# smartroboticslab/okvis2

Measured on AMD Instinct MI355X. Metric: front-end stereo-frames/s (detect+describe+match), 752x480 stereo, higher is better.
Workload: dtype u8/int32 (detect, describe, Hamming) + f64 (match gate); 1 GPU; EuRoC-shaped 752x480 stereo, euroc.yaml front-end params (radius 38, thr 150, <=700 kpts, match thr 60); lanes_per_gpu=1, score_kernels_serialised_across_lanes=False, stereo_frames_per_launch=3072, distinct_frames=256, content=corners, feed=device, cameras_per_multiframe=2, parallelism=frames sharded over 1 GPU(s), no collective

## Files before the change

okvis2_amd/csrc/describe_setup_dev.h:

```cpp
#pragma once
#include "okvfe_internal.h"

namespace okvfe {

__device__ __forceinline__ bool camera_aware_matrix(const float* __restrict__ rays,
                                                    const float* __restrict__ jac, int w, float fu,
                                                    const float dir[3], float kx, float ky,
                                                    float M[4]) {
  const int u = (int)(kx + 0.5f), v = (int)(ky + 0.5f);
  const float* r = rays + ((size_t)v * w + u) * 3;
  const float* J = jac + ((size_t)v * w + u) * 6;
  const float r0 = r[0], r1 = r[1], r2 = r[2];
  if (r0 == 0.0f && r1 == 0.0f && r2 == 0.0f) return false;
  float ey0 = 0.f, ey1 = 0.f, ey2 = 0.f, n2 = 0.0f;
#pragma unroll
  for (int c = 0; c < 3; ++c) {
    const float g0 = c == 0 ? dir[0] : (c == 1 ? 0.0f : 1.0f);
    const float g1 = c == 0 ? dir[1] : (c == 1 ? 1.0f : 0.0f);
    const float g2 = c == 0 ? dir[2] : 0.0f;
    if (c > 0 && n2 >= 1.0e-12f) break;
    float gr = g0 * r0;
    float t = g1 * r1;
    gr = gr + t;
    t = g2 * r2;
    gr = gr + t;
    t = gr * r0; ey0 = g0 - t;
    t = gr * r1; ey1 = g1 - t;
    t = gr * r2; ey2 = g2 - t;
    n2 = ey0 * ey0;
    t = ey1 * ey1;
    n2 = n2 + t;
    t = ey2 * ey2;
    n2 = n2 + t;
  }
  if (!(n2 >= 1.0e-12f)) return false;
  const float n = sqrtf(n2);
  ey0 = ey0 / n;
  ey1 = ey1 / n;
  ey2 = ey2 / n;
  float t1, t2;
  t1 = ey1 * r2; t2 = ey2 * r1; const float ex0 = t1 - t2;
  t1 = ey2 * r0; t2 = ey0 * r2; const float ex1 = t1 - t2;
  t1 = ey0 * r1; t2 = ey1 * r0; const float ex2 = t1 - t2;
  float s;
  s = J[0] * ex0; t1 = J[1] * ex1; s = s + t1; t1 = J[2] * ex2; s = s + t1; M[0] = s / fu;
  s = J[0] * ey0; t1 = J[1] * ey1; s = s + t1; t1 = J[2] * ey2; s = s + t1; M[1] = s / fu;
  s = J[3] * ex0; t1 = J[4] * ex1; s = s + t1; t1 = J[5] * ex2; s = s + t1; M[2] = s / fu;
  s = J[3] * ey0; t1 = J[4] * ey1; s = s + t1; t1 = J[5] * ey2; s = s + t1; M[3] = s / fu;
  return true;
}

template <int MAXB2>
__device__ __forceinline__ bool extra_sample_value(const uint8_t* __restrict__ im, int w, int h, float xf, float yf,
                                                   float sigma_half, int scaling, int scaling2, int* value) {
  const float x_1 = xf - sigma_half, x1 = xf + sigma_half;
  const float y_1 = yf - sigma_half, y1 = yf + sigma_half;
  if (!(x_1 >= 0.0f && y_1 >= 0.0f && x1 < (float)(w - 1) && y1 < (float)(h - 1))) return false;
  const int x_left = (int)(x_1 + 0.5f), y_top = (int)(y_1 + 0.5f);
  const int x_right = (int)(x1 + 0.5f), y_bottom = (int)(y1 + 0.5f);
  float r_x_1 = (float)x_left - x_1;  r_x_1 = r_x_1 + 0.5f;
  float r_y_1 = (float)y_top - y_1;   r_y_1 = r_y_1 + 0.5f;
  float r_x1 = x1 - (float)x_right;   r_x1 = r_x1 + 0.5f;
  float r_y1 = y1 - (float)y_bottom;  r_y1 = r_y1 + 0.5f;
  const float fs = (float)scaling;
  float t;
  t = r_x_1 * r_y_1; const int A = (int)(t * fs);
  t = r_x1 * r_y_1;  const int B = (int)(t * fs);
  t = r_x1 * r_y1;   const int C = (int)(t * fs);
  t = r_x_1 * r_y1;  const int D = (int)(t * fs);
  const int r_x_1_i = (int)(r_x_1 * fs), r_y_1_i = (int)(r_y_1 * fs);
  const int r_x1_i = (int)(r_x1 * fs), r_y1_i = (int)(r_y1 * fs);
  const int bw = x_right - x_left, bh = y_bottom - y_top;
  if (bw > MAXB2 || bh > MAXB2) return false;
  constexpr int NDW = (3 + MAXB2) / 4 + 1;
  const int b = x_left & 3;
  const uint8_t* p0 = im + (size_t)y_top * w + (x_left & ~3);
  auto byte_at = [&](const uint32_t (&r)[NDW], int pos) -> int {
    uint32_t v = r[0];
#pragma unroll
    for (int j = 1; j < NDW; ++j) v = (pos >> 2) == j ? r[j] : v;
    return (int)((v >> (8 * (pos & 3))) & 0xFFu);
  };
  uint32_t msk[NDW];
#pragma unroll
  for (int j = 0; j < NDW; ++j) {
    int lo = b + 1 - 4 * j, hi = b + bw - 4 * j;
    lo = lo < 0 ? 0 : (lo > 4 ? 4 : lo);
    hi = hi < 0 ? 0 : (hi > 4 ? 4 : hi);
    const uint32_t mlo = lo >= 4 ? 0xFFFFFFFFu : ((1u << (8 * lo)) - 1u);
    const uint32_t mhi = hi >= 4 ? 0xFFFFFFFFu : ((1u << (8 * hi)) - 1u);
    msk[j] = mhi & ~mlo;
  }
  int upper = 0, middle = 0, left = 0, right = 0, bottom = 0, pl_t = 0, pr_t = 0, pl_b = 0, pr_b = 0;
  constexpr int kChunk = 5;
#pragma unroll
  for (int c0 = 0; c0 <= MAXB2; c0 += kChunk) {
    uint32_t d[kChunk][NDW];
#pragma unroll
    for (int r = 0; r < kChunk; ++r) {
      const int dy = c0 + r;
      if (dy <= MAXB2) {
        const uint32_t* q = reinterpret_cast<const uint32_t*>(p0 + (size_t)(dy < bh ? dy : bh) * w);
#pragma unroll
        for (int j = 0; j < NDW; ++j) d[r][j] = q[j];
      }
    }
#pragma unroll
    for (int r = 0; r < kChunk; ++r) {
      const int dy = c0 + r;
      if (dy <= MAXB2) {
        const int pl = byte_at(d[r], b), pr = byte_at(d[r], b + bw);
        int in = 0;
#pragma unroll
        for (int j = 0; j < NDW; ++j) in += (int)__builtin_amdgcn_sad_u8(d[r][j] & msk[j], 0u, 0u);
        if (dy == 0) {
          pl_t = pl;
          pr_t = pr;
          upper = in;
        } else if (dy < bh) {
          left += pl;
          right += pr;
          middle += in;
        } else if (dy == bh) {
          pl_b = pl;
          pr_b = pr;
          bottom = in;
        }
      }
    }
  }
  int ret = A * pl_t;
  ret += B * pr_t;
  ret += C * pr_b;
  ret += D * pl_b;
  ret += upper * r_y_1_i + middle * scaling + left * r_x_1_i + right * r_x1_i + bottom * r_y1_i;
  *value = (ret + scaling2 / 2) / scaling2;
  return true;
}

__device__ __forceinline__ bool extra_sample_one(const Pattern* __restrict__ pat, const uint8_t* __restrict__ im, int w,
                                                 int h, int extra_box, int e, const float M[4], float kx, float ky,
                                                 uint8_t* __restrict__ slot_bytes) {
  const float px = pat->px[e], py = pat->py[e], sg = pat->sigma_half[e];
  float a = M[0] * px, b2 = M[1] * py;
  a = a + b2;
  const float xf = kx + a;
  float c = M[2] * px, d2 = M[3] * py;
  c = c + d2;
  const float yf = ky + c;
  int v = 0;
  const bool ok = extra_box <= 4
                      ? extra_sample_value<4>(im, w, h, xf, yf, sg, pat->box_scaling[e], pat->box_scaling2[e], &v)
                      : extra_sample_value<9>(im, w, h, xf, yf, sg, pat->box_scaling[e], pat->box_scaling2[e], &v);
  *reinterpret_cast<int*>(slot_bytes + 24 + 4 * e) = v;
  return ok;
}

__device__ __forceinline__ void describe_setup_one(const DescribeSetup& ds, int w, int h, int img, size_t slot,
                                                   const okvfe_keypoint& kp) {
  const ImageParams ip = ds.prm[img];
  int scale = 0;
  if (ds.scales) {
    for (int i = 1; i < kPatternScales; ++i) scale += kp.size >= ds.scales->size_from[i] ? 1 : 0;
  }
// ... 51 lines not shown
```

okvis2_amd/csrc/k_select.hip:

```cpp
#include <mutex>
#include "describe_setup_dev.h"
#include <type_traits>

#include "select_common_dev.h"

namespace okvfe {
namespace {

constexpr int kLazyTabBytes = 32 * 32 * 4;
constexpr int kLazyThreads = 256;
constexpr int kLazyBinCap = 4;
#ifndef OKVFE_LAZY_BLOCKMAX
#define OKVFE_LAZY_BLOCKMAX 1024
#endif
#ifndef OKVFE_LAZY_WAVES
#define OKVFE_LAZY_WAVES 6
#endif
constexpr int kLazyBlockMax = OKVFE_LAZY_BLOCKMAX;
constexpr int kLazySurvPerWave = kLazyBlockMax / 4;
__host__ __device__ inline size_t lazy_align16(size_t v) { return (v + 15) & ~(size_t)15; }
__host__ __device__ inline size_t lazy_lds_bytes(int bins_x, int bins_y) {
  const size_t nbins = (size_t)(bins_x + 2) * (bins_y + 2);
  return (size_t)kLazyTabBytes + lazy_align16(nbins * 4) + nbins * kLazyBinCap * 8 + (size_t)kLazyBlockMax * 8 +
         4 * 64 * 4;
}

__device__ __forceinline__ void lds_barrier() {
  asm volatile("s_waitcnt lgkmcnt(0)\n\ts_barrier" ::: "memory");
}

#ifdef OKVFE_LAB
__device__ unsigned long long g_lazy_prof[16];
#define OKVFE_LAZY_TICK(var) const unsigned long long var = __builtin_amdgcn_s_memrealtime()
#else
#define OKVFE_LAZY_TICK(var)
#endif
constexpr int kFuseBins = 496;
constexpr int kFuseUnroll = 8;
constexpr int kFuseFirst = 20;
constexpr int kFuseSched = 40;
__device__ __forceinline__ int fuse_bin(int32_t score) {
  if (score <= 0) return kFuseBins - 1;
  const uint32_t s = (uint32_t)score;
  const int e = 31 - __clz(s);
  const int b = e >= 4 ? (e << 4) | (int)((s >> (e - 4)) & 15u) : (int)s;
  return (kFuseBins - 1) - b;
}
template <bool SORTS>
__global__ __launch_bounds__(kLazyThreads) __attribute__((amdgpu_waves_per_eu(OKVFE_LAZY_WAVES, 8))) void select_lazy_kernel(
    const int32_t* __restrict__ scores, ScoreLayout layout, int w, int h, const Candidate* __restrict__ cand, int cand_cap,
    const int32_t* __restrict__ cand_count, uint64_t* sort_ws, int ws_stride,
    float radius, int max_kpts, const float* __restrict__ lut, int bins_x, int bins_y, int cap,
    okvfe_keypoint* __restrict__ kps, int kp_cap, int32_t* __restrict__ kp_count, uint2* __restrict__ spill_ws,
    size_t spill_stride, int bin_cap, int round_cap, DescribeSetup setup, const uint8_t* __restrict__ images) {
  extern __shared__ __attribute__((aligned(16))) unsigned char smem_raw[];
  __shared__ int s_kept;
  __shared__ int s_spill;
  __shared__ int s_surv[2][4];
  __shared__ uint32_t s_sched[kFuseSched + 2];
  __shared__ int s_nsched, s_max, s_cnt;
  __shared__ unsigned long long s_kmin, s_kmax;
  const int bpitch = bins_x + 2;
  const int nbins = bpitch * (bins_y + 2);
  float* tab = reinterpret_cast<float*>(smem_raw);
  unsigned char* q0 = smem_raw + kLazyTabBytes;
  uint32_t* head = reinterpret_cast<uint32_t*>(q0);
  q0 += lazy_align16((size_t)nbins * 4);
  uint4* slot4 = reinterpret_cast<uint4*>(q0);
  q0 += (size_t)nbins * kLazyBinCap * 8;
  uint64_t* surv = reinterpret_cast<uint64_t*>(q0);
  float* part = reinterpret_cast<float*>(q0 + (size_t)kLazyBlockMax * 8);
  const int tid = threadIdx.x;
  const int wave = __builtin_amdgcn_readfirstlane(tid >> 6);
  const int lane = tid & 63;
  const int img = blockIdx.x;
  int n = cand_count[img];
  n = n > cand_cap ? 0 : n;
  uint64_t* keys = sort_ws + (size_t)img * ws_stride;
  okvfe_keypoint* out = kps + (size_t)img * kp_cap;
  uint2* spill = spill_ws + (size_t)img * spill_stride;
  int kept = 0;
  OKVFE_LAZY_TICK(t_start);
#ifdef OKVFE_LAB
  unsigned long long t_pa = t_start, t_pb = t_start, t_p0 = t_start, t_init = t_start, t_blocks = t_start, t_pref = 0, t_mark = 0, t_walk = 0, t_acc = 0, t_ins = 0, t_w0 = 0, t_w1 = 0, t_w2 = 0;
  int n_surv = 0, n_rounds = 0;
#endif
  if (n > 0) {
    for (int i = tid; i < 32 * 32; i += kLazyThreads) {
      const int dx = i & 31, dy = i >> 5;
      tab[i] = (dx <= 15 && dy <= 15) ? lut[(dy + 15) * 31 + (dx + 15)] : 0.0f;
    }
    for (int i = tid; i < nbins; i += kLazyThreads) head[i] = 0u;
    for (int i = tid; i < nbins * 2; i += kLazyThreads)
      slot4[i] = make_uint4((16u << 23) | (16u << 2), 0u, (16u << 23) | (16u << 2), 0u);
    if (tid == 0) {
      s_kept = 0;
      s_spill = 0;
      if constexpr (SORTS) s_max = INT_MIN;
    }
    if constexpr (SORTS) {
      for (int i = tid; i <= kFuseBins; i += kLazyThreads) reinterpret_cast<uint32_t*>(surv)[i] = 0u;
    }
    const Candidate* crec = cand + (size_t)img * cand_cap;
    int32_t scv0[SORTS ? kFuseFirst : 1];
    uint32_t pyx0[SORTS ? kFuseFirst : 1];
    if constexpr (SORTS) {
#pragma unroll
      for (int u = 0; u < kFuseFirst; ++u) {
        const int i = tid + u * kLazyThreads;
        const Candidate c = i < n ? crec[i] : Candidate{0, 0, INT_MIN};
        scv0[u] = c.score;
        pyx0[u] = ((uint32_t)c.y << 16) | (uint32_t)c.x;
      }
    }
    const float scaling = (float)(15.0 / (double)radius);
    float max_score = 1.0f;
    if constexpr (!SORTS) max_score = (float)(0x7FFFFFFF - (int32_t)(keys[0] >> 32));
    auto make_rec = [&](uint64_t k) {
      const int score = 0x7FFFFFFF - (int32_t)(k >> 32);
      const int y = (int)((k >> 16) & 0xFFFF), x = (int)(k & 0xFFFF);
      const float fy = (float)y * scaling;
      const float fx = (float)x * scaling;
      const int cy = (int)(fy + 16.0f);
      const int cx = (int)(fx + 16.0f);
      const float q = (float)score / max_score;
      const float nsc1 = sqrtf(sqrtf(q)) * 255.0f;
      return make_uint4(((uint32_t)cy << 16) | (uint32_t)cx, __float_as_uint(nsc1), (uint32_t)(k & 0xFFFFFFFFu),
                        (uint32_t)score);
    };
    const uint32_t tab_addr = (uint32_t)(uintptr_t)(__attribute__((address_space(3))) float*)tab;
    auto waddr_of = [&](uint32_t A, uint32_t code, uint32_t levbits) {
      const uint32_t a = __builtin_amdgcn_sad_u16(A, code, tab_addr);
      return levbits != 0u ? a : tab_addr;
    };
    auto term = [&](uint32_t waddr, uint32_t levbits) {
      return ceilf(*reinterpret_cast<__attribute__((address_space(3))) const float*>((uintptr_t)waddr) *
                   __uint_as_float(levbits));
    };
    auto bins3 = [&](const int b[3], const uint32_t A[3], int half) {
      uint4 s3[3];
#pragma unroll
      for (int k = 0; k < 3; ++k) s3[k] = slot4[2 * b[k] + half];
      uint32_t wa[6];
#pragma unroll
      for (int k = 0; k < 3; ++k) {
        wa[2 * k] = waddr_of(A[k], half == 0 ? s3[k].x & ~1u : s3[k].x, s3[k].y);
        wa[2 * k + 1] = waddr_of(A[k], s3[k].z, s3[k].w);
      }
      float f = 0.0f;
#pragma unroll
      for (int k = 0; k < 3; ++k) f += term(wa[2 * k], s3[k].y) + term(wa[2 * k + 1], s3[k].w);
      return f;
    };
    auto spill_terms = [&](int cx, int cy) {
      float f = 0.0f;
      const int ns = s_spill;
      for (int i = 0; i < ns; ++i) {
        const uint2 p = spill[i];
        const int dx = cx - (int)(p.x & 0xFFFF), dy = cy - (int)(p.x >> 16);
        const int adx = dx < 0 ? -dx : dx, ady = dy < 0 ? -dy : dy;
        if (adx <= 15 && ady <= 15) f += ceilf(tab[(ady << 5) | adx] * __uint_as_float(p.y));
      }
      return f;
    };
    const int first = (wave + 1) & 3;
    const int nch = first == 0 ? 3 : 2;
    int hoff[3];
    uint32_t aoff[3];
#pragma unroll
    for (int k = 0; k < 3; ++k) {
      const int c = first + 4 * k < 9 ? first + 4 * k : first;
      const int ox = (c % 3) - 1, oy = (c / 3) - 1;
      hoff[k] = oy * bpitch + ox;
      aoff[k] = ((uint32_t)(-16 * oy) << 23) + ((uint32_t)(-16 * ox) << 2);
    }
    const int limit = min(min(max_kpts, kp_cap), cap);
    uint64_t* my_surv = surv + wave * kLazySurvPerWave;
    auto prefilter_key = [&](uint64_t kthis, bool valid) -> bool {
          uint4 rec = make_rec(kthis);
          if (!valid) rec.x = 0u;
          const int cx = (int)(rec.x & 0xFFFF), cy = (int)(rec.x >> 16);
          const float level = __uint_as_float(rec.y);
          const int bin = ((cy >> 4) + 1) * bpitch + ((cx >> 4) + 1);
          const uint32_t lx = (uint32_t)(cx & 15), ly = (uint32_t)(cy & 15);
          const uint32_t A0 = ((ly + 16u) << 23) | ((lx + 16u) << 2);
          float occf = 0.0f;
          {
            bool more = false;
            auto batch = [&](auto first, auto count) {
              constexpr int B0 = decltype(first)::value, NB = decltype(count)::value;
              uint32_t A[NB];
              uint4 sb[NB];
#pragma unroll
              for (int q = 0; q < NB; ++q) {
                const int b = B0 + q;
// ... 196 lines not shown
#pragma unroll
        for (int t = 0; t < 4; ++t) {
          const int i = lo + 64 * t + lane;
          kr[t] = i < hi ? keys[i] : 0ull;
        }
      };
      uint64_t kcur[4] = {0ull, 0ull, 0ull, 0ull}, knxt[4];
      int blen = 64, par = 0;
      for (int a = 0; a < n; a += blen, blen = min(2 * blen, kLazyBlockMax), par ^= 1) {
        const int e = min(a + blen, n);
#ifdef OKVFE_LAB
        t_mark = __builtin_amdgcn_s_memrealtime();
#endif
        int my_cnt = 0;
        if (a == 0) {
          const int q = (e - a + 3) >> 2;
          const int lo = wave * q, hi = min(lo + q, e - a);
          for (int c = lo + lane; c < hi; c += 64) my_surv[c - lo] = keys[c];
          my_cnt = hi > lo ? hi - lo : 0;
        } else {
          const int q = blen >> 2;
          const int lo = a + wave * q, hi = min(lo + q, e);
#pragma unroll
          for (int t = 0; t < 4; ++t) {
            const int c0 = lo + 64 * t;
            if (c0 >= hi) break;
            const uint64_t kthis = kcur[t];
            const bool pass = prefilter_key(kthis, c0 + lane < hi);
            const unsigned long long m = __ballot(pass);
            if (pass) my_surv[my_cnt + __popcll(m & ((1ull << lane) - 1ull))] = kthis;
            my_cnt += __popcll(m);
          }
        }
        load_quarter(a + blen, min(2 * blen, kLazyBlockMax), knxt);
        if (lane == 0) s_surv[par][wave] = my_cnt;
        lds_barrier();
        const int c0n = s_surv[par][0], c1n = c0n + s_surv[par][1], c2n = c1n + s_surv[par][2],
                  total = c2n + s_surv[par][3];
#ifdef OKVFE_LAB
        n_surv += total;
        t_pref += __builtin_amdgcn_s_memrealtime() - t_mark;
#endif
        windows(total, [&](int g) {
          int li = 0, lo = g;
          if (g >= c2n) { li = 3; lo = g - c2n; }
          else if (g >= c1n) { li = 2; lo = g - c1n; }
          else if (g >= c0n) { li = 1; lo = g - c0n; }
          return surv[li * kLazySurvPerWave + lo];
        });
        if (kept >= limit) break;
#pragma unroll
        for (int t = 0; t < 4; ++t) kcur[t] = knxt[t];
      }
    } else {
      uint32_t* hist = reinterpret_cast<uint32_t*>(surv);
      __syncthreads();
#ifdef OKVFE_LAB
      t_p0 = __builtin_amdgcn_s_memrealtime();
#endif
      {
        int mx = INT_MIN;
#pragma unroll
        for (int u = 0; u < kFuseFirst; ++u) {
          if (tid + u * kLazyThreads < n) {
            atomicAdd(&hist[fuse_bin(scv0[u])], 1u);
            mx = max(mx, scv0[u]);
          }
        }
        for (int base = tid + kFuseFirst * kLazyThreads; base < n; base += 8 * kLazyThreads) {
          int32_t scv[8];
#pragma unroll
          for (int u = 0; u < 8; ++u) {
            const int i = base + u * kLazyThreads;
            scv[u] = i < n ? crec[i].score : INT_MIN;
          }
#pragma unroll
          for (int u = 0; u < 8; ++u) {
            if (base + u * kLazyThreads < n) {
              atomicAdd(&hist[fuse_bin(scv[u])], 1u);
              mx = max(mx, scv[u]);
            }
          }
        }
#pragma unroll
        for (int d = 32; d > 0; d >>= 1) mx = max(mx, __shfl_xor(mx, d));
        if (lane == 0) atomicMax(&s_max, mx);
      }
      __syncthreads();
#ifdef OKVFE_LAB
      t_pa = __builtin_amdgcn_s_memrealtime();
#endif
      max_score = (float)s_max;
      if (wave == 0) {
        uint32_t v[8], sum = 0;
#pragma unroll
        for (int k = 0; k < 8; ++k) {
          const int idx = lane * 8 + k;
          v[k] = idx < kFuseBins ? hist[idx] : 0u;
          sum += v[k];
        }
        uint32_t inc = sum;
#pragma unroll
        for (int d = 1; d < 64; d <<= 1) {
          const uint32_t t = __shfl_up(inc, d);
          if (lane >= d) inc += t;
        }
        uint32_t run = inc - sum;
        __builtin_amdgcn_wave_barrier();
#pragma unroll
        for (int k = 0; k < 8; ++k) {
          const int idx = lane * 8 + k;
          if (idx <= kFuseBins) hist[idx] = run;
          run += v[k];
        }
        __builtin_amdgcn_wave_barrier();
        int pos = 0, b = 0, k = 0;
        uint32_t target = min(64u, (uint32_t)round_cap);
        while (pos < n && k < kFuseSched) {
          int x_last = b - 1;
          for (int base = b; base < kFuseBins; base += 64) {
            const int idx = base + lane;
            const uint32_t ve = idx < kFuseBins ? hist[idx + 1] : 0xFFFFFFFFu;
            const bool ok = idx < kFuseBins && ve - (uint32_t)pos <= target;
            const int c = __popcll(__ballot(ok));
            x_last += c;
            if (c < 64) break;
          }
          int e = x_last >= b ? (int)hist[x_last + 1] : pos;
          if (e == pos) {
            for (int base = b; base < kFuseBins; base += 64) {
              const int idx = base + lane;
              const bool gt = idx < kFuseBins && (int)hist[idx + 1] > pos;
              const unsigned long long m = __ballot(gt);
              if (m != 0ull) {
                x_last = base + (int)__ffsll((long long)m) - 1;
                break;
              }
            }
            e = (int)hist[x_last + 1];
          }
          if (lane == 0) s_sched[k] = (uint32_t)e;
          ++k;
          pos = e;
          b = x_last + 1;
          target = min(2u * target, (uint32_t)round_cap);
        }
        if (pos < n) {
          if (lane == 0) s_sched[k] = (uint32_t)n;
          ++k;
        }
        if (lane == 0) s_nsched = k;
      }
      __syncthreads();
#ifdef OKVFE_LAB
      t_pb = __builtin_amdgcn_s_memrealtime();
#endif
#pragma unroll
      for (int u = 0; u < kFuseFirst; ++u) {
        if (tid + u * kLazyThreads < n) {
          const uint32_t p = atomicAdd(&hist[fuse_bin(scv0[u])], 1u);
          keys[p] = ((uint64_t)(uint32_t)(0x7FFFFFFF - scv0[u]) << 32) | pyx0[u];
        }
      }
      for (int base = tid + kFuseFirst * kLazyThreads; base < n; base += kFuseUnroll * kLazyThreads) {
        Candidate cv[kFuseUnroll];
#pragma unroll
        for (int u = 0; u < kFuseUnroll; ++u) {
          const int i = base + u * kLazyThreads;
          cv[u] = i < n ? crec[i] : Candidate{0, 0, 0};
        }
#pragma unroll
        for (int u = 0; u < kFuseUnroll; ++u) {
          if (base + u * kLazyThreads < n) {
            const uint32_t p = atomicAdd(&hist[fuse_bin(cv[u].score)], 1u);
            keys[p] = make_key(cv[u]);
          }
        }
      }
      __syncthreads();
#ifdef OKVFE_LAB
      t_init = __builtin_amdgcn_s_memrealtime();
#endif
      const int nsched = s_nsched;
      uint64_t kcur[4] = {0ull, 0ull, 0ull, 0ull}, knxt[4] = {0ull, 0ull, 0ull, 0ull};
      auto load_chunk = [&](int c0, int m, uint64_t kr[4]) {
        const int q = (m + 3) >> 2;
        const int lo = c0 + wave * q, hi = min(lo + q, c0 + m);
#pragma unroll
        for (int t = 0; t < 4; ++t) {
          const int i = lo + 64 * t + lane;
          kr[t] = i < hi ? keys[i] : 0ull;
        }
      };
      int cpos = 0, j = 0, par = 0;
      bool have_next = false;
      bool refining = false;
      int r_base = 0, r_m = 0, r_rem = 0;
      uint64_t r_lo = 0ull;
      while (true) {
        int cnt = 0;
#ifdef OKVFE_LAB
        t_mark = __builtin_amdgcn_s_memrealtime();
#endif
        if (!refining) {
          if (j >= nsched) break;
          const int e = (int)s_sched[j];
          const int m = e - cpos;
          ++j;
          if (m > round_cap) {
            refining = true;
            r_base = cpos; r_m = m; r_rem = m; r_lo = 0ull;
            cpos = e;
            have_next = false;
            continue;
          }
          if (have_next) {
#pragma unroll
            for (int t = 0; t < 4; ++t) kcur[t] = knxt[t];
          } else {
            load_chunk(cpos, m, kcur);
          }
          cnt = m;
          cpos = e;
          have_next = false;
        } else {
          uint64_t hi = ~0ull;
          if (r_rem > round_cap) {
            if (tid == 0) {
              s_kmin = ~0ull;
              s_kmax = 0ull;
            }
            __syncthreads();
            unsigned long long mn = ~0ull, mxk = 0ull;
            for (int i = tid; i < r_m; i += kLazyThreads) {
              const unsigned long long k = keys[r_base + i];
              if (k >= r_lo) {
                mn = k < mn ? k : mn;
                mxk = k > mxk ? k : mxk;
              }
            }
#pragma unroll
            for (int d = 32; d > 0; d >>= 1) {
              const unsigned long long a1 = __shfl_xor(mn, d), a2 = __shfl_xor(mxk, d);
              mn = a1 < mn ? a1 : mn;
              mxk = a2 > mxk ? a2 : mxk;
            }
            if (lane == 0) {
              atomicMin(&s_kmin, mn);
              atomicMax(&s_kmax, mxk);
            }
            __syncthreads();
            const unsigned long long kmin = s_kmin, range = s_kmax - kmin;
            int sh = range < 256ull ? 0 : (64 - __clzll((long long)range)) - 8;
            uint32_t* sub = reinterpret_cast<uint32_t*>(part);
            while (true) {
              sub[tid] = 0u;
              __syncthreads();
              for (int i = tid; i < r_m; i += kLazyThreads) {
                const unsigned long long k = keys[r_base + i];
                if (k >= r_lo) {
                  const unsigned long long d = (k - kmin) >> sh;
                  if (d < 256ull) atomicAdd(&sub[(int)d], 1u);
                }
              }
              __syncthreads();
              uint32_t v4[4], sum = 0;
#pragma unroll
              for (int k = 0; k < 4; ++k) {
                v4[k] = sub[lane * 4 + k];
                sum += v4[k];
              }
              uint32_t inc = sum;
#pragma unroll
              for (int d = 1; d < 64; d <<= 1) {
                const uint32_t t = __shfl_up(inc, d);
                if (lane >= d) inc += t;
              }
              uint32_t run = inc - sum;
              int nfit = 0;
#pragma unroll
              for (int k = 0; k < 4; ++k) {
                run += v4[k];
                nfit += __popcll(__ballot(run <= (uint32_t)round_cap));
              }
              __syncthreads();
              if (nfit == 0 && sh > 0) {
                sh = sh >= 8 ? sh - 8 : 0;
                continue;
              }
              hi = kmin + ((unsigned long long)(nfit > 0 ? nfit : 1) << sh);
              break;
            }
          }
          if (tid == 0) s_cnt = 0;
          __syncthreads();
          for (int i0 = 0; i0 < r_m; i0 += kLazyThreads) {
            const int i = i0 + tid;
            const unsigned long long k = i < r_m ? keys[r_base + i] : 0ull;
            const bool pred = i < r_m && k >= r_lo && k < hi;
            const unsigned long long m = __ballot(pred);
            if (m != 0ull) {
              int base = 0;
              if (lane == 0) base = atomicAdd(&s_cnt, __popcll(m));
              base = __builtin_amdgcn_readfirstlane(base);
              const int at = base + __popcll(m & ((1ull << lane) - 1ull));
              if (pred && at < kLazyBlockMax) surv[at] = k;
            }
          }
          __syncthreads();
          const int got = s_cnt;
          cnt = got < kLazyBlockMax ? got : kLazyBlockMax;
          {
            const int q = (cnt + 3) >> 2;
            const int lo = wave * q, hi_i = min(lo + q, cnt);
#pragma unroll
            for (int t = 0; t < 4; ++t) {
              const int i = lo + 64 * t + lane;
              kcur[t] = i < hi_i ? surv[i] : 0ull;
            }
          }
          __syncthreads();
          r_rem -= got;
          r_lo = hi;
          if (r_rem <= 0 || got == 0) refining = false;
        }
        int my_cnt = 0;
        {
          const int q = (cnt + 3) >> 2;
          const int lo = wave * q, hi_i = min(lo + q, cnt);
#pragma unroll
          for (int t = 0; t < 4; ++t) {
            const int c0 = lo + 64 * t;
            if (c0 >= hi_i) break;
            const uint64_t kthis = kcur[t];
            const bool valid = c0 + lane < hi_i;
            const bool pass = kept > 0 ? prefilter_key(kthis, valid) : valid;
            const unsigned long long m = __ballot(pass);
            if (pass) my_surv[my_cnt + __popcll(m & ((1ull << lane) - 1ull))] = kthis;
            my_cnt += __popcll(m);
          }
        }
        if (!refining && j < nsched) {
          const int m2 = (int)s_sched[j] - cpos;
          if (m2 <= round_cap) {
            load_chunk(cpos, m2, knxt);
            have_next = true;
          }
        }
        int* racc = reinterpret_cast<int*>(part);
        racc[tid] = 0;
        if (lane == 0) s_surv[par][wave] = my_cnt;
        lds_barrier();
        const int c0n = s_surv[par][0], c1n = c0n + s_surv[par][1], c2n = c1n + s_surv[par][2],
                  total = c2n + s_surv[par][3];
        par ^= 1;
#ifdef OKVFE_LAB
        n_surv += total;
        ++n_rounds;
#endif
        auto list_key = [&](int g) {
          int li = 0, lo = g;
          if (g >= c2n) { li = 3; lo = g - c2n; }
          else if (g >= c1n) { li = 2; lo = g - c1n; }
          else if (g >= c0n) { li = 1; lo = g - c0n; }
          return surv[li * kLazySurvPerWave + lo];
        };
        auto list_len = [&](int w2) { return w2 == 0 ? c0n : (w2 == 1 ? c1n - c0n : (w2 == 2 ? c2n - c1n : total - c2n)); };
        if (total <= kLazyThreads / 2) {
          const int per = total <= 64 ? 1 : 2;
          const int g = total <= 64 ? lane : (tid & 127);
          const int w0 = total <= 64 ? wave : 2 * (wave >> 1);
          const uint64_t mykey = g < total ? list_key(g) : ~0ull;
          int r = 0;
          for (int w2 = w0; w2 < w0 + per; ++w2) {
            const uint64_t* lst = surv + w2 * kLazySurvPerWave;
            const int c = list_len(w2);
#pragma unroll 8
            for (int jj = 0; jj < c; ++jj) r += lst[jj] < mykey ? 1 : 0;
          }
          if (g < total && r != 0) atomicAdd(&racc[g], r);
          lds_barrier();
          if (w0 == 0 && g < total) surv[racc[g]] = mykey;
          lds_barrier();
        } else {
          const int nu = (total + kLazyThreads - 1) / kLazyThreads;
          uint64_t mykey[4];
          int rank[4];
#pragma unroll
          for (int u = 0; u < 4; ++u) {
            const int g = tid + u * kLazyThreads;
            mykey[u] = (u < nu && g < total) ? list_key(g) : ~0ull;
            rank[u] = 0;
          }
#pragma unroll
          for (int w2 = 0; w2 < 4; ++w2) {
            const uint64_t* lst = surv + w2 * kLazySurvPerWave;
            const int c = list_len(w2);
            if (nu <= 1) {
#pragma unroll 8
              for (int jj = 0; jj < c; ++jj) rank[0] += lst[jj] < mykey[0] ? 1 : 0;
            } else {
              for (int jj = 0; jj < c; ++jj) {
                const uint64_t k2 = lst[jj];
#pragma unroll
                for (int u = 0; u < 4; ++u) rank[u] += k2 < mykey[u] ? 1 : 0;
              }
            }
          }
          lds_barrier();
#pragma unroll
          for (int u = 0; u < 4; ++u)
            if (u < nu && tid + u * kLazyThreads < total) surv[rank[u]] = mykey[u];
          lds_barrier();
        }
#ifdef OKVFE_LAB
        t_pref += __builtin_amdgcn_s_memrealtime() - t_mark;
#endif
        windows(total, [&](int g) { return surv[g]; });
        if (kept >= limit) break;
      }
    }
  }
  __syncthreads();
#ifdef OKVFE_LAB
  t_blocks = __builtin_amdgcn_s_memrealtime();
#endif
  for (int i = tid; i < kept; i += kLazyThreads) {
    okvfe_keypoint kp = out[i];
    const int u = (int)kp.x, v = (int)kp.y;
    int32_t patch[9];
    if (images) {
      harris_scores_3x3(images + (size_t)img * w * h, w, h, u, v, patch);
    } else {
      const int32_t* sc = scores + (size_t)img * layout.pitch * h;
#pragma unroll
      for (int dy = -1; dy <= 1; ++dy)
#pragma unroll
        for (int dx = -1; dx <= 1; ++dx)
          patch[(dy + 1) * 3 + (dx + 1)] = sc[score_index(layout, u + dx, v + dy)];
    }
    float ddx, ddy;
    subpixel2d(patch, &ddx, &ddy);
    kp.x = (float)u + ddx;
    kp.y = (float)v + ddy;
    kp.response = (float)kp.class_id;
    kp.class_id = -1;
    out[i] = kp;
    if (setup.pat) describe_setup_one(setup, w, h, img, (size_t)img * kp_cap + i, kp);
  }
  if (tid == 0) kp_count[img] = kept;
#ifdef OKVFE_LAB
  __syncthreads();
  if (tid == 0 && img == 0) {
    const unsigned long long t_end = __builtin_amdgcn_s_memrealtime();
    atomicAdd(&g_lazy_prof[0], 1ull);
    atomicAdd(&g_lazy_prof[1], t_init - t_start);
    atomicAdd(&g_lazy_prof[2], t_blocks - t_init);
    atomicAdd(&g_lazy_prof[3], t_end - t_blocks);
    atomicAdd(&g_lazy_prof[4], t_end - t_start);
    atomicAdd(&g_lazy_prof[5], t_pref);
    atomicAdd(&g_lazy_prof[6], (unsigned long long)n_surv);
    atomicAdd(&g_lazy_prof[7], (unsigned long long)n);
    atomicAdd(&g_lazy_prof[8], t_walk);
    atomicAdd(&g_lazy_prof[9], t_acc);
    atomicAdd(&g_lazy_prof[10], t_ins);
    atomicAdd(&g_lazy_prof[11], (unsigned long long)n_rounds);
    atomicAdd(&g_lazy_prof[12], t_p0 - t_start);
    atomicAdd(&g_lazy_prof[13], t_pa - t_p0);
    atomicAdd(&g_lazy_prof[14], t_pb - t_pa);
    atomicAdd(&g_lazy_prof[15], t_init - t_pb);
  }
#endif
}

}


constexpr int kListChunk = 128;
constexpr int kListLutBytes = 64 * 64 * 4;
__device__ __forceinline__ uint32_t lds_u32(uint32_t addr) {
  return *reinterpret_cast<__attribute__((address_space(3))) const uint32_t*>((uintptr_t)addr);
}
__device__ __forceinline__ float lds_f32(uint32_t addr) {
  return *reinterpret_cast<__attribute__((address_space(3))) const float*>((uintptr_t)addr);
}
__host__ __device__ inline size_t list_lds_bytes(int bins_x, int bins_y, int cap) {
  return (size_t)kListLutBytes + lazy_align16((size_t)(bins_x + 2) * (bins_y + 2) * 4) +
         2 * lazy_align16((size_t)(cap + 1) * 4) + (size_t)kListChunk * 16 + 4 * 64 * 4;
}

__global__ __launch_bounds__(kLazyThreads) __attribute__((amdgpu_waves_per_eu(6, 8))) void select_list_kernel(
    const int32_t* __restrict__ scores, ScoreLayout layout, int w, int h, int cand_cap,
    const int32_t* __restrict__ cand_count, const uint64_t* __restrict__ sort_ws, int ws_stride,
    float radius, int max_kpts, const float* __restrict__ lut, int bins_x, int bins_y, int cap,
    okvfe_keypoint* __restrict__ kps, int kp_cap, int32_t* __restrict__ kp_count, DescribeSetup setup,
    const uint8_t* __restrict__ images) {
  extern __shared__ __attribute__((aligned(16))) unsigned char smem_raw[];
  __shared__ int s_kept;
  const int bpitch = bins_x + 2;
  const int nbins = bpitch * (bins_y + 2);
  const size_t cap4 = lazy_align16((size_t)(cap + 1) * 4);
  float* lut_s = reinterpret_cast<float*>(smem_raw);
  unsigned char* q0 = smem_raw + kListLutBytes;
  uint32_t* head = reinterpret_cast<uint32_t*>(q0);
  q0 += lazy_align16((size_t)nbins * 4);
  uint32_t* link = reinterpret_cast<uint32_t*>(q0);
  float* pnsc = reinterpret_cast<float*>(q0 + cap4);
  uint4* recs = reinterpret_cast<uint4*>(q0 + 2 * cap4);
  float* part = reinterpret_cast<float*>(q0 + 2 * cap4 + (size_t)kListChunk * 16);
  const int tid = threadIdx.x;
  const int wave = __builtin_amdgcn_readfirstlane(tid >> 6);
  const int lane = tid & 63;
  const int img = blockIdx.x;
  int n = cand_count[img];
  n = n > cand_cap ? 0 : n;
  const uint64_t* keys = sort_ws + (size_t)img * ws_stride;
  okvfe_keypoint* out = kps + (size_t)img * kp_cap;
  int kept = 0;
  if (n > 0) {
    for (int i = tid; i < 64 * 64; i += kLazyThreads) {
      const int dx = (i & 63) - 32, dy = (i >> 6) - 32;
      const bool in = dx >= -15 && dx <= 15 && dy >= -15 && dy <= 15;
      lut_s[i] = in ? lut[(dy + 15) * 31 + (dx + 15)] : 0.0f;
    }
    const uint32_t link_addr = (uint32_t)(uintptr_t)(__attribute__((address_space(3))) uint32_t*)link;
    const uint32_t end_addr = link_addr + 4u * (uint32_t)cap;
    const uint32_t nsc_delta = (uint32_t)cap4;
    const uint32_t lut_addr = (uint32_t)(uintptr_t)(__attribute__((address_space(3))) float*)lut_s;
    for (int i = tid; i < nbins; i += kLazyThreads) head[i] = end_addr;
    if (tid == 0) {
      pnsc[cap] = 0.0f;
      link[cap] = (end_addr >> 2) << 16;
// ... 99 lines not shown
            if (!pass) cm = 0ull;
            unsigned long long nb = 0ull;
            while (__any(cm != 0ull)) {
              const int el = cm != 0ull ? (int)__ffsll((long long)cm) - 1 : lane;
              const uint32_t exy = (uint32_t)__builtin_amdgcn_ds_bpermute(el << 2, (int)rec.x);
              if (cm != 0ull) {
                cm &= cm - 1ull;
                const uint32_t ddx = (uint32_t)(cx - (int)(exy & 0xFFFF) + 15);
                const uint32_t ddy = (uint32_t)(cy - (int)(exy >> 16) + 15);
                nb |= (ddx <= 30u && ddy <= 30u) ? (1ull << el) : 0ull;
              }
            }
            while (rem != 0ull) {
              const bool in = ((rem >> lane) & 1ull) != 0ull;
              const bool ready = in && (nb & rem) == 0ull;
              const unsigned long long rdy = __ballot(ready);
              const unsigned long long accn = __ballot(ready && pass);
              accm |= accn;
              rem &= ~rdy;
              unsigned long long m = (in && !ready) ? (nb & accn) : 0ull;
              while (__any(m != 0ull)) {
                const int jl = m != 0ull ? (int)__ffsll((long long)m) - 1 : lane;
                const uint32_t jxy = (uint32_t)__builtin_amdgcn_ds_bpermute(jl << 2, (int)rec.x);
                const float jnsc = __int_as_float(__builtin_amdgcn_ds_bpermute(jl << 2, __float_as_int(nsc)));
                if (m != 0ull) {
                  m &= m - 1ull;
                  const int dx = cx - (int)(jxy & 0xFFFF), dy = cy - (int)(jxy >> 16);
                  occ += (int)ceilf(lut_s[((dy + 32) << 6) | (dx + 32)] * jnsc);
                }
              }
              if (in && !ready) pass = !(level < (float)(occ > 255 ? 255 : occ));
              rem &= __ballot(pass);
            }
            nacc = __popcll(accm);
          } else {
            while (rem != 0 && kept + nacc < limit) {
              const int f = (int)__ffsll((long long)rem) - 1;
              accm |= 1ull << f;
              ++nacc;
              const uint32_t wxy = (uint32_t)__builtin_amdgcn_readlane((int)rec.x, f);
              const float wnsc = __int_as_float(__builtin_amdgcn_readlane(__float_as_int(nsc), f));
              const int dx = cx - (int)(wxy & 0xFFFF), dy = cy - (int)(wxy >> 16);
              const bool near = pass && lane > f && (dx < 0 ? -dx : dx) <= 15 && (dy < 0 ? -dy : dy) <= 15;
              if (__any(near)) {
                if (near) {
                  occ += (int)ceilf(lut_s[((dy + 32) << 6) | (dx + 32)] * wnsc);
                  pass = !(level < (float)(occ > 255 ? 255 : occ));
                }
                rem &= __ballot(pass) & ~(((2ull << f) - 1ull));
              } else {
                rem &= rem - 1;
              }
            }
          }
          if ((accm >> lane) & 1) {
            const int slot = kept + __popcll(accm & ((1ull << lane) - 1ull));
            const uint32_t addr = link_addr + 4u * (uint32_t)slot;
            const uint32_t prev = atomicExch(&head[bin], addr);
            link[slot] = (lcode << 2) | ((prev >> 2) << 16);
            pnsc[slot] = nsc;
            okvfe_keypoint kp;
            kp.x = (float)(int)(rec.z & 0xFFFF);
            kp.y = (float)(int)(rec.z >> 16);
            kp.size = 12.0f;
            kp.angle = -1.0f;
            kp.response = (float)(int32_t)rec.w;
            kp.octave = 0;
            kp.class_id = (int32_t)rec.w;
            out[slot] = kp;
          }
          kept += nacc;
          if (lane == 0) s_kept = kept;
        }
      } else if (((pos + 64) & (kListChunk - 1)) == 0) {
        convert();
        request(pos + 64 + kListChunk);
      }
      lds_barrier();
      kept = s_kept;
      if (kept >= limit) break;
    }
  }
  __syncthreads();
  for (int i = tid; i < kept; i += kLazyThreads) {
    okvfe_keypoint kp = out[i];
    const int u = (int)kp.x, v = (int)kp.y;
    int32_t patch[9];
    if (images) {
      harris_scores_3x3(images + (size_t)img * w * h, w, h, u, v, patch);
    } else {
      const int32_t* sc = scores + (size_t)img * layout.pitch * h;
#pragma unroll
      for (int dy = -1; dy <= 1; ++dy)
#pragma unroll
        for (int dx = -1; dx <= 1; ++dx)
          patch[(dy + 1) * 3 + (dx + 1)] = sc[score_index(layout, u + dx, v + dy)];
    }
    float ddx, ddy;
    subpixel2d(patch, &ddx, &ddy);
    kp.x = (float)u + ddx;
    kp.y = (float)v + ddy;
    kp.response = (float)kp.class_id;
    kp.class_id = -1;
    out[i] = kp;
    if (setup.pat) describe_setup_one(setup, w, h, img, (size_t)img * kp_cap + i, kp);
  }
  if (tid == 0) kp_count[img] = kept;
}

namespace {
struct LazyPlan {
  bool list, array;
  int bins_x, bins_y, cap;
  size_t lds, lds_list;
};
constexpr size_t kLazyMaxLds = 159 * 1024;
LazyPlan lazy_plan(float radius, int max_kpts, int kp_cap, const uint8_t* occupancy, size_t occ_image_bytes,
                   int occ_rows, int occ_cols) {
  LazyPlan p{};
  static const bool legacy = lab_env("OKVFE_LEGACY_SELECT") != nullptr;
  static const bool grid = lab_env("OKVFE_SELECT_GRID") != nullptr;
  if (!(radius > 0.0f) || legacy || grid || occ_cols > 65535 || occ_rows > 65535) return p;
  p.bins_x = (occ_cols + 15) >> 4;
  p.bins_y = (occ_rows + 15) >> 4;
  p.cap = max_kpts < kp_cap ? max_kpts : kp_cap;
  p.lds = lazy_lds_bytes(p.bins_x, p.bins_y);
  p.lds_list = list_lds_bytes(p.bins_x, p.bins_y, p.cap);
  const bool array_ok = p.lds <= kLazyMaxLds && occupancy != nullptr && occ_image_bytes >= (size_t)p.cap * 8;
  const bool prefer_list = !array_ok || (p.lds > 48 * 1024 && kLazyMaxLds / p.lds_list > kLazyMaxLds / p.lds);
  p.list = prefer_list && p.lds_list <= kLazyMaxLds;
  p.array = !p.list && array_ok;
  return p;
}
bool lazy_presorted() {
  static const bool v = lab_env("OKVFE_SELECT_PRESORTED") != nullptr;
  return v;
}
}

bool select_recomputes_scores(float radius, int max_kpts, int kp_cap, const uint8_t* occupancy, size_t occ_image_bytes,
                              int occ_rows, int occ_cols) {
  const LazyPlan p = lazy_plan(radius, max_kpts, kp_cap, occupancy, occ_image_bytes, occ_rows, occ_cols);
  return p.array || p.list;
}
bool select_sorts_candidates(float radius, int max_kpts, int kp_cap, const uint8_t* occupancy, size_t occ_image_bytes,
                             int occ_rows, int occ_cols) {
  return lazy_plan(radius, max_kpts, kp_cap, occupancy, occ_image_bytes, occ_rows, occ_cols).array && !lazy_presorted();
}

bool launch_select(const int32_t* score, ScoreLayout layout, int w, int h, int n_images, Candidate* cand,
                   int cand_cap, const int32_t* cand_count, float radius, int max_kpts,
                   const float* lut, uint8_t* occupancy, size_t occ_image_bytes, int occ_rows,
                   int occ_cols, okvfe_keypoint* kps, int kp_cap, int32_t* kp_count,
                   uint64_t* sort_ws, hipStream_t stream, const DescribeSetup* setup, const uint8_t* images) {
  if (n_images <= 0) return false;
  int ws_stride = 1;
  while (ws_stride < cand_cap) ws_stride <<= 1;
  const LazyPlan lp = lazy_plan(radius, max_kpts, kp_cap, occupancy, occ_image_bytes, occ_rows, occ_cols);
  if (lp.list) {
    static PerDeviceOnce attr_once_l;
    attr_once_l.run([] {
      if (hipFuncSetAttribute(reinterpret_cast<const void*>(select_list_kernel),
                              hipFuncAttributeMaxDynamicSharedMemorySize, (int)kLazyMaxLds) != hipSuccess)
        (void)hipGetLastError();
    });
    hipLaunchKernelGGL(select_list_kernel, dim3(n_images), dim3(kLazyThreads), lp.lds_list, stream, score, layout, w, h,
                       cand_cap, cand_count, sort_ws, ws_stride, radius, max_kpts, lut, lp.bins_x, lp.bins_y, lp.cap, kps,
                       kp_cap, kp_count, setup ? *setup : DescribeSetup{}, images);
    return setup != nullptr;
  }
  if (lp.array) {
    static const int bin_cap = [] {
      const char* e = lab_env("OKVFE_LAZY_BINCAP");
      const int v = e ? atoi(e) : kLazyBinCap;
      return v < 1 ? 1 : (v > kLazyBinCap ? kLazyBinCap : v);
    }();
    static const int round_cap = [] {
      const char* e = lab_env("OKVFE_LAZY_ROUNDCAP");
      const int v = e ? atoi(e) : kLazyBlockMax;
      return v < 4 ? 4 : (v > kLazyBlockMax ? kLazyBlockMax : v);
    }();
    static PerDeviceOnce attr_once;
    attr_once.run([] {
      if (hipFuncSetAttribute(reinterpret_cast<const void*>(select_lazy_kernel<true>),
                              hipFuncAttributeMaxDynamicSharedMemorySize, (int)kLazyMaxLds) != hipSuccess)
        (void)hipGetLastError();
      if (hipFuncSetAttribute(reinterpret_cast<const void*>(select_lazy_kernel<false>),
                              hipFuncAttributeMaxDynamicSharedMemorySize, (int)kLazyMaxLds) != hipSuccess)
        (void)hipGetLastError();
// ... 31 lines not shown
```

Measured before the change: 719,200 stereo-frames/s.

## Micro-optimize select kernel: binary byte select, drop wave reductions, branchless chunk loads

Several unrelated micro-edits. The linear byte_at select becomes a log-depth binary mux. Candidate x/y fields are packed with 16-bit vector loads. Per-wave shuffle reductions before the LDS atomics are replaced by direct per-lane atomicMax/Min. Chunk key loads are made branchless with clamped indices, and the duplicated refine/emit loop is factored into a helper. Per-lane LDS atomics can serialize more than the shuffle tree they replace, and the clamped loads read duplicate keys, which relies on the downstream code ignoring them.

```diff
diff --git a/okvis2_amd/csrc/describe_setup_dev.h b/okvis2_amd/csrc/describe_setup_dev.h
--- a/okvis2_amd/csrc/describe_setup_dev.h
+++ b/okvis2_amd/csrc/describe_setup_dev.h
@@ -76,10 +76,16 @@
   const int b = x_left & 3;
   const uint8_t* p0 = im + (size_t)y_top * w + (x_left & ~3);
   auto byte_at = [&](const uint32_t (&r)[NDW], int pos) -> int {
-    uint32_t v = r[0];
-#pragma unroll
-    for (int j = 1; j < NDW; ++j) v = (pos >> 2) == j ? r[j] : v;
-    return (int)((v >> (8 * (pos & 3))) & 0xFFu);
+    uint32_t v[NDW];
+#pragma unroll
+    for (int j = 0; j < NDW; ++j) v[j] = r[j];
+#pragma unroll
+    for (int bit = 0; (1 << bit) < NDW; ++bit) {
+      const bool hi = ((pos >> (2 + bit)) & 1) != 0;
+#pragma unroll
+      for (int j = 0; j + (1 << bit) < NDW; j += 2 << bit) v[j] = hi ? v[j + (1 << bit)] : v[j];
+    }
+    return (int)((v[0] >> (8 * (pos & 3))) & 0xFFu);
   };
   uint32_t msk[NDW];
 #pragma unroll
diff --git a/okvis2_amd/csrc/k_select.hip b/okvis2_amd/csrc/k_select.hip
--- a/okvis2_amd/csrc/k_select.hip
+++ b/okvis2_amd/csrc/k_select.hip
@@ -6,6 +6,32 @@
 
 namespace okvfe {
 namespace {
+
+__device__ __forceinline__ void refine_emit(const int32_t* __restrict__ scores, const ScoreLayout& layout, int w, int h,
+                                            int img, const uint8_t* __restrict__ images, const DescribeSetup& setup,
+                                            okvfe_keypoint* __restrict__ out, int i, size_t slot) {
+  okvfe_keypoint kp = out[i];
+  const int u = (int)kp.x, v = (int)kp.y;
+  int32_t patch[9];
+  if (images) {
+    harris_scores_3x3(images + (size_t)img * w * h, w, h, u, v, patch);
+  } else {
+    const int32_t* sc = scores + (size_t)img * layout.pitch * h;
+#pragma unroll
+    for (int dy = -1; dy <= 1; ++dy)
+#pragma unroll
+      for (int dx = -1; dx <= 1; ++dx)
+        patch[(dy + 1) * 3 + (dx + 1)] = sc[score_index(layout, u + dx, v + dy)];
+  }
+  float ddx, ddy;
+  subpixel2d(patch, &ddx, &ddy);
+  kp.x = (float)u + ddx;
+  kp.y = (float)v + ddy;
+  kp.response = (float)kp.class_id;
+  kp.class_id = -1;
+  out[i] = kp;
+  if (setup.pat) describe_setup_one(setup, w, h, img, slot, kp);
+}
 
 constexpr int kLazyTabBytes = 32 * 32 * 4;
 constexpr int kLazyThreads = 256;
@@ -105,12 +131,21 @@
     int32_t scv0[SORTS ? kFuseFirst : 1];
     uint32_t pyx0[SORTS ? kFuseFirst : 1];
     if constexpr (SORTS) {
+      typedef unsigned short ushort2_t __attribute__((ext_vector_type(2)));
 #pragma unroll
       for (int u = 0; u < kFuseFirst; ++u) {
         const int i = tid + u * kLazyThreads;
-        const Candidate c = i < n ? crec[i] : Candidate{0, 0, INT_MIN};
-        scv0[u] = c.score;
-        pyx0[u] = ((uint32_t)c.y << 16) | (uint32_t)c.x;
+        if (i < n) {
+          const unsigned short* c16 = reinterpret_cast<const unsigned short*>(crec + i);
+          ushort2_t yx;
+          yx.x = c16[0];
+          yx.y = c16[2];
+          pyx0[u] = __builtin_bit_cast(uint32_t, yx);
+          scv0[u] = crec[i].score;
+        } else {
+          pyx0[u] = 0u;
+          scv0[u] = INT_MIN;
+        }
       }
     }
     const float scaling = (float)(15.0 / (double)radius);
@@ -473,9 +508,7 @@
             }
           }
         }
-#pragma unroll
-        for (int d = 32; d > 0; d >>= 1) mx = max(mx, __shfl_xor(mx, d));
-        if (lane == 0) atomicMax(&s_max, mx);
+        atomicMax(&s_max, mx);
       }
       __syncthreads();
 #ifdef OKVFE_LAB
@@ -576,12 +609,9 @@
       uint64_t kcur[4] = {0ull, 0ull, 0ull, 0ull}, knxt[4] = {0ull, 0ull, 0ull, 0ull};
       auto load_chunk = [&](int c0, int m, uint64_t kr[4]) {
         const int q = (m + 3) >> 2;
-        const int lo = c0 + wave * q, hi = min(lo + q, c0 + m);
-#pragma unroll
-        for (int t = 0; t < 4; ++t) {
-          const int i = lo + 64 * t + lane;
-          kr[t] = i < hi ? keys[i] : 0ull;
-        }
+        const int lo = c0 + wave * q;
+#pragma unroll
+        for (int t = 0; t < 4; ++t) kr[t] = keys[min(lo + 64 * t + lane, c0 + m - 1)];
       };
       int cpos = 0, j = 0, par = 0;
       bool have_next = false;
@@ -630,16 +660,8 @@
                 mxk = k > mxk ? k : mxk;
               }
             }
-#pragma unroll
-            for (int d = 32; d > 0; d >>= 1) {
-              const unsigned long long a1 = __shfl_xor(mn, d), a2 = __shfl_xor(mxk, d);
-              mn = a1 < mn ? a1 : mn;
-              mxk = a2 > mxk ? a2 : mxk;
-            }
-            if (lane == 0) {
-              atomicMin(&s_kmin, mn);
-              atomicMax(&s_kmax, mxk);
-            }
+            atomicMin(&s_kmin, mn);
+            atomicMax(&s_kmax, mxk);
             __syncthreads();
             const unsigned long long kmin = s_kmin, range = s_kmax - kmin;
             int sh = range < 256ull ? 0 : (64 - __clzll((long long)range)) - 8;
@@ -731,11 +753,14 @@
             my_cnt += __popcll(m);
           }
         }
-        if (!refining && j < nsched) {
-          const int m2 = (int)s_sched[j] - cpos;
-          if (m2 <= round_cap) {
+        {
+          const int m2 = !refining && j < nsched ? (int)s_sched[j] - cpos : 0;
+          have_next = m2 > 0 && m2 <= round_cap;
+          if (have_next) {
             load_chunk(cpos, m2, knxt);
-            have_next = true;
+          } else {
+#pragma unroll
+            for (int t = 0; t < 4; ++t) knxt[t] = 0ull;
           }
         }
         int* racc = reinterpret_cast<int*>(part);
@@ -816,29 +841,8 @@
 #ifdef OKVFE_LAB
   t_blocks = __builtin_amdgcn_s_memrealtime();
 #endif
-  for (int i = tid; i < kept; i += kLazyThreads) {
-    okvfe_keypoint kp = out[i];
-    const int u = (int)kp.x, v = (int)kp.y;
-    int32_t patch[9];
-    if (images) {
-      harris_scores_3x3(images + (size_t)img * w * h, w, h, u, v, patch);
-    } else {
-      const int32_t* sc = scores + (size_t)img * layout.pitch * h;
-#pragma unroll
-      for (int dy = -1; dy <= 1; ++dy)
-#pragma unroll
-        for (int dx = -1; dx <= 1; ++dx)
-          patch[(dy + 1) * 3 + (dx + 1)] = sc[score_index(layout, u + dx, v + dy)];
-    }
-    float ddx, ddy;
-    subpixel2d(patch, &ddx, &ddy);
-    kp.x = (float)u + ddx;
-    kp.y = (float)v + ddy;
-    kp.response = (float)kp.class_id;
-    kp.class_id = -1;
-    out[i] = kp;
-    if (setup.pat) describe_setup_one(setup, w, h, img, (size_t)img * kp_cap + i, kp);
-  }
+  for (int i = tid; i < kept; i += kLazyThreads)
+    refine_emit(scores, layout, w, h, img, images, setup, out, i, (size_t)img * kp_cap + i);
   if (tid == 0) kp_count[img] = kept;
 #ifdef OKVFE_LAB
   __syncthreads();
@@ -1104,29 +1108,8 @@
     }
   }
   __syncthreads();
-  for (int i = tid; i < kept; i += kLazyThreads) {
-    okvfe_keypoint kp = out[i];
-    const int u = (int)kp.x, v = (int)kp.y;
-    int32_t patch[9];
-    if (images) {
-      harris_scores_3x3(images + (size_t)img * w * h, w, h, u, v, patch);
-    } else {
-      const int32_t* sc = scores + (size_t)img * layout.pitch * h;
-#pragma unroll
-      for (int dy = -1; dy <= 1; ++dy)
-#pragma unroll
-        for (int dx = -1; dx <= 1; ++dx)
-          patch[(dy + 1) * 3 + (dx + 1)] = sc[score_index(layout, u + dx, v + dy)];
-    }
-    float ddx, ddy;
-    subpixel2d(patch, &ddx, &ddy);
-    kp.x = (float)u + ddx;
-    kp.y = (float)v + ddy;
-    kp.response = (float)kp.class_id;
-    kp.class_id = -1;
-    out[i] = kp;
-    if (setup.pat) describe_setup_one(setup, w, h, img, (size_t)img * kp_cap + i, kp);
-  }
+  for (int i = tid; i < kept; i += kLazyThreads)
+    refine_emit(scores, layout, w, h, img, images, setup, out, i, (size_t)img * kp_cap + i);
   if (tid == 0) kp_count[img] = kept;
 }
 
```

After: 736,100 stereo-frames/s, median of 6. 2.3% higher.
